# thodson-usgs/discontinuum

Measured on AMD Instinct MI355X. Metric: GP fits/sec (NLL+grad step) at n=8192 d=3, 1/2/4/8 MI355X, higher is better.
Workload: dtype f64

## Files before the change

### discontinuum_amd/_lib.py

```python
from __future__ import annotations

import ctypes as C
import os

_HERE = os.path.dirname(os.path.abspath(__file__))
LIB_PATH = os.path.join(_HERE, "libdgp_hip.so")

F64, F32 = 0, 1
MODEL_LOADEST, MODEL_RATING = 0, 1
OUT_NLL, OUT_QUAD, OUT_LOGDET, OUT_INFO, OUT_DTHETA, OUT_SUM_DR, OUT_DR_W0, OUT_SUM_DNOISE, OUT_LEN = 0, 1, 2, 3, 4, 28, 29, 31, 32
BUF_XT, BUF_A, BUF_T, BUF_S, BUF_Z, BUF_ALPHA = range(6)
BUF_INFO, BUF_SCAL = 6, 7
LCV_PLANE_NAMES = ("mu", "var", "lpd", "pit_lower", "pit_upper", "dlp", "tilt")
OPT_LAUUM64_MAX_TILES, OPT_SYRK_SLOTS, OPT_TRTRI_SMALL, OPT_REFINE, OPT_SYRK_ORDER, OPT_LAUUM_ORDER, OPT_CHAIN_YIELD, OPT_FUSED_GRAD, OPT_GROUP_GEMM = range(9)
OPT_POTRF_SCHEDULE, OPT_POTRF_SWEEP, OPT_POTRF_SOLVE, OPT_POTRF_OVERLAP, OPT_POTRF_SLOTS, OPT_POTRF_TAIL, OPT_POTRF_TAIL_SWEEP = range(9, 16)
TIME_GRAM, TIME_POTRF, TIME_SYRK_SUM, TIME_SYRK_N, TIME_TRTRI, TIME_LAUUM, TIME_SOLVE, TIME_GRAD, TIME_SYRK_FLOP, TIME_COUNT = range(10)


E_ARG, E_MODEL, E_WORKSPACE, E_STATE, E_FULL, E_NOCONV = -1, -2, -3, -4, -5, -6


class DGPLibraryError(RuntimeError):
    pass

# ... 89 lines not shown
    "dgp_predict_sensitivity_workspace_bytes": (_sz, [_vp, _i64, _i, _i]),
    "dgp_predict_sensitivity": (_i, [_vp, _dp, _vp, _i64, _vp, _i, _vp, _i, _vp, _sz, _vp, _vp, _vp]),
    "dgp_deletion_influence_workspace_bytes": (_sz, [_vp, _i64, _i, _i64, _i]),
    "dgp_deletion_influence": (_i, [_vp, _dp, _vp, _i64, _vp, _vp, _i, _i64, _i, _vp, _vp, _vp, _i, _vp, _vp, _sz, _vp, _vp, _vp, _vp, _vp]),
    "dgp_model_nterms": (_i, [_i, _i]),
    "dgp_predict_terms_workspace_bytes": (_sz, [_vp, _i64]),
    "dgp_predict_terms": (_i, [_vp, _dp, _vp, _i64, _vp, _sz, _vp, _vp, _vp]),
    "dgp_model_input_differentiable": (_i, [_i, _i, _i]),
    "dgp_predict_slopes_workspace_bytes": (_sz, [_vp, _i64, _i]),
    "dgp_predict_slopes": (_i, [_vp, _dp, _vp, _i64, C.POINTER(_i), _i, _vp, _sz, _vp, _vp, _vp]),
    "dgp_mean_vjp_workspace_bytes": (_sz, [_vp, _i64]),
    "dgp_predict_mean": (_i, [_vp, _dp, _vp, _i64, _vp, _sz, _vp, _vp]),
    "dgp_mean_vjp": (_i, [_vp, _dp, _vp, _i64, _vp, _vp, _sz, _vp, _vp, _vp, _vp]),
    "dgp_plan_set_timing": (_i, [_vp, _i]),
    "dgp_plan_get_timing": (_i, [_vp, _dp]),
    "dgp_stage_gram": (_i, [_vp, _dp, _vp, _vp]),
    "dgp_stage_potrf": (_i, [_vp, _vp]),
    "dgp_stage_trtri": (_i, [_vp, _vp]),
    "dgp_stage_lauum": (_i, [_vp, _vp]),
    "dgp_stage_solve": (_i, [_vp, _vp, _vp]),
    "dgp_stage_grad": (_i, [_vp, _dp, _vp, _vp]),
    "dgp_cross_gram": (_i, [_vp, _dp, _vp, _i64, _vp, _vp, _vp]),
    "dgp_debug_clock_probe": (_i, [_vp, _i, C.c_double, _vp]),
    "dgp_debug_tile_gemm": (_i, [_i, _i, _i, _i, _vp, _i64, _vp, _i64, _i64, _vp, _i64, _i, _i, _i, _i, _vp]),
}

_lib = None


def load():
    global _lib
    if _lib is not None:
        return _lib
    if not os.path.exists(LIB_PATH):
        raise DGPLibraryError(
            f"{LIB_PATH} not found: build it with `python -c 'import __graft_entry__ as g; g.build()'` "
            "or `make -C discontinuum_amd/csrc` (there is no CPU fallback)"
        )
    try:
        lib = C.CDLL(LIB_PATH)
    except OSError as e:
        raise DGPLibraryError(f"could not load {LIB_PATH}: {e}") from e
    for name, (res, args) in SIGNATURES.items():
        fn = getattr(lib, name)
        fn.restype = res
        fn.argtypes = args
# ... 10 lines not shown
```

### discontinuum_amd/csrc/dgp_chol.hip

```cpp
#include <stdlib.h>
#include <string.h>
#include <algorithm>
#include <mutex>
#include "dgp_diag.h"
#include "dgp_gemm.h"
#include "dgp_gemm_dma.h"
#include "dgp_internal.h"
#include "dgp_schedule.h"

namespace dgp {

static constexpr int NB = DGP_TILE;
static constexpr int SMID_TABLE = 4096;
template <typename T>
struct Prefetch {
  static constexpr bool F64 = sizeof(T) == 8;
  static constexpr int LAUUM = F64 ? 2 : 4, TRTRI = F64 ? 1 : 4, SYRK = F64 ? 1 : 2;
};

#define DGP_INFO_CHAIN_TIMEOUT (-7)
#define CHAIN_WAIT_TICKS 200000000LL
__device__ __forceinline__ bool chain_reached(const int* word, int value) {
  return __hip_atomic_load(word, __ATOMIC_RELAXED, __HIP_MEMORY_SCOPE_AGENT) >= value;
}
// ... 913 lines not shown
  G::foreach (acc, [&](int r, int c, T& v) { out[(long)r * ld + c] = v; });
}

template <typename T>
int lauum(const T* Tm, long N, T* S, hipStream_t s, Batch bt) {
  const int nbk = (int)(N / NB);
  const int tiles = nbk * (nbk + 1) / 2;
  if ((long)tiles * bt.B <= bt.tuning().lauum64_max_tiles) {
    const int nb64 = 2 * nbk;
    lauum64_kernel<T><<<dim3((unsigned)(nb64 * (nb64 + 1) / 2), 1, (unsigned)bt.B), 256, 0, s>>>(Tm, S, N, nb64, bt.ws);
  } else {
    const int sup = bt.tuning().lauum_super;
    unsigned grid = (unsigned)tiles;
    if (sup > 0) {
      const int nsr = (nbk + sup - 1) / sup, nst = nsr * (nsr + 1) / 2;
      grid = (unsigned)((nst + 7) / 8 * 8 * sup * sup);
    }
    lauum_kernel<T><<<dim3(grid, 1, (unsigned)bt.B), 256, 0, s>>>(Tm, S, N, nbk, bt.ws, sup);
  }
  return (int)hipGetLastError();
}

template <typename T>
__global__ __launch_bounds__(256) void trmv_n_kernel(const T* __restrict__ Tm, long ld, const T* __restrict__ r, int n,
                                                     T* __restrict__ z, long bs, const int* __restrict__ ns, long rs,
                                                     long zs = -1 ) {
  Tm = site(Tm, bs);
  z = site(z, zs >= 0 ? zs : bs);
  r = site(r, rs);
  n = site_n(ns, n);
  const int lane = threadIdx.x & 63;
  const long i = (long)blockIdx.x * 4 + (threadIdx.x >> 6);
  const long jend = (i / NB + 1) * NB;
  const T* row = Tm + i * ld;
  T acc = T(0);
  for (long j = lane; j < jend; j += 64) acc += row[j] * (j < n ? r[j] : T(0));
  acc = wave_sum(acc);
  if (lane == 0) z[i] = acc;
}

#define DGP_TRMV_CHUNK 512
static inline int trmv_chunk(long N) { return N < 2048 ? 128 : DGP_TRMV_CHUNK; }
template <typename T>
__global__ __launch_bounds__(256) void trmv_t_kernel(const T* __restrict__ Tm, long ld, const T* __restrict__ z,
                                                     T* __restrict__ partial, long bs, int chunk, long zs = -1) {
  Tm = site(Tm, bs);
  z = site(z, zs >= 0 ? zs : bs);
  partial = site(partial, zs >= 0 ? zs : bs);
  __shared__ T red[4][64];
  const int tx = threadIdx.x & 63, ty = threadIdx.x >> 6;
  const long j = (long)blockIdx.x * 64 + tx;
  const long r0 = (long)blockIdx.y * chunk, r1 = min(r0 + (long)chunk, ld);
  const long rstart = max(r0, ((long)blockIdx.x * 64 / NB) * NB);
  T acc = T(0);
  for (long i = rstart + ty; i < r1; i += 4) acc += Tm[i * ld + j] * z[i];
  red[ty][tx] = acc;
  __syncthreads();
  if (ty == 0) partial[(long)blockIdx.y * ld + j] = red[0][tx] + red[1][tx] + red[2][tx] + red[3][tx];
}

template <typename T>
__global__ __launch_bounds__(256) void trmv_t_reduce_kernel(const T* __restrict__ partial, long N, int nchunks,
                                                            T* __restrict__ alpha, long bs, int chunk,
                                                            const T* __restrict__ z, T* __restrict__ quad, long as = -1,
                                                            long zs = -1 ) {
  if (zs >= 0) bs = zs;
  if (blockIdx.x == gridDim.x - 1) {
    if (quad == nullptr) return;
    z = site(z, bs);
    quad = site(quad, bs);
    __shared__ double red[256];
    double acc = 0.0;
    for (long i = threadIdx.x; i < N; i += 256) acc += (double)z[i] * (double)z[i];
    red[threadIdx.x] = acc;
    __syncthreads();
    for (int s = 128; s > 0; s >>= 1) {
      if ((int)threadIdx.x < s) red[threadIdx.x] += red[threadIdx.x + s];
      __syncthreads();
    }
    if (threadIdx.x == 0) {
      quad[0] = (T)red[0];
      if (sizeof(T) == 4) *reinterpret_cast<double*>(quad + 3) = red[0];
    }
    return;
  }
  partial = site(partial, bs);
  alpha = site(alpha, as >= 0 ? as : bs);
  const long j = (long)blockIdx.x * 256 + threadIdx.x;
  if (j >= N) return;
  T acc = T(0);
  const int c0 = (int)((j / NB) * NB / chunk);
  for (int c = c0; c < nchunks; ++c) acc += partial[(long)c * N + j];
  alpha[j] = acc;
}

template <typename T>
__global__ __launch_bounds__(256) void symv_row_kernel(const T* __restrict__ S, long ld, const T* __restrict__ g,
                                                       T* __restrict__ out, long bs, long wbs) {
  S = site(S, bs);
  g = site(g, wbs);
  out = site(out, wbs);
  const int lane = threadIdx.x & 63;
  const long i = (long)blockIdx.x * 4 + (threadIdx.x >> 6);
  const T* row = S + i * ld;
  T acc = T(0);
  for (long j = lane; j <= i; j += 64) acc += row[j] * g[j];
  acc = wave_sum(acc);
  if (lane == 0) out[i] = acc;
}
template <typename T>
__global__ __launch_bounds__(256) void symv_col_kernel(const T* __restrict__ S, long ld, const T* __restrict__ g,
                                                       T* __restrict__ partial, long bs, long wbs) {
  S = site(S, bs);
  g = site(g, wbs);
  partial = site(partial, wbs);
  __shared__ T red[4][64];
  const int tx = threadIdx.x & 63, ty = threadIdx.x >> 6;
  const long j = (long)blockIdx.x * 64 + tx;
// ... 17 lines not shown
  n = site_n(ns, n);
  const long j = (long)blockIdx.x * 256 + threadIdx.x;
  if (j >= N) return;
  T acc = beta[j];
  for (int c = (int)(j / DGP_TRMV_CHUNK); c < nchunks; ++c) acc += partial[(long)c * N + j];
  acc = j < n ? acc : T(0);
  beta[j] = acc;
  if (j < nfull && dnoise) dnoise[j] = j < n ? -acc * alpha[j] : T(0);
}

template <typename T>
int symv_lower(const T* S, long N, const T* g, int n, const T* alpha, T* beta, T* partials, T* dnoise, hipStream_t s,
               Batch bt, long wbs) {
  const int nchunks = (int)((N + DGP_TRMV_CHUNK - 1) / DGP_TRMV_CHUNK);
  const unsigned Bz = (unsigned)bt.B;
  symv_row_kernel<T><<<dim3((unsigned)(N / 4), 1, Bz), 256, 0, s>>>(S, N, g, beta, bt.ws, wbs);
  dim3 grid((unsigned)(N / 64), (unsigned)nchunks, Bz);
  symv_col_kernel<T><<<grid, 256, 0, s>>>(S, N, g, partials, bt.ws, wbs);
  symv_finish_kernel<T><<<dim3((unsigned)((N + 255) / 256), 1, Bz), 256, 0, s>>>(partials, N, nchunks, alpha, n, beta, dnoise, bt.ws,
                                                                                wbs, bt.ns);
  return (int)hipGetLastError();
}

long solve_partials(long N) { return (N + trmv_chunk(N) - 1) / trmv_chunk(N) * N; }

template <typename T>
static void solve_pair(const T* Tm, long N, const T* r, long rs, int n, T* z, T* out, long os, T* partials, T* quad, hipStream_t s,
                       const Batch& bt) {
  const unsigned Bz = (unsigned)bt.B;
  trmv_n_kernel<T><<<dim3((unsigned)(N / 4), 1, Bz), 256, 0, s>>>(Tm, N, r, n, z, bt.ws, bt.ns, rs);
  const int chunk = trmv_chunk(N), nchunks = (int)((N + chunk - 1) / chunk);
  dim3 grid((unsigned)(N / 64), (unsigned)nchunks, Bz);
  trmv_t_kernel<T><<<grid, 256, 0, s>>>(Tm, N, z, partials, bt.ws, chunk);
  trmv_t_reduce_kernel<T><<<dim3((unsigned)((N + 255) / 256) + 1, 1, Bz), 256, 0, s>>>(partials, N, nchunks, out, bt.ws, chunk, z, quad, os);
}
template <typename T>
int solve(const T* Tm, long N, const T* r, int n, T* z, T* alpha, T* partials, T* quad, hipStream_t s, Batch bt) {
  solve_pair<T>(Tm, N, r, (long)n, n, z, alpha, -1, partials, quad, s, bt);
  return (int)hipGetLastError();
}
template <typename T>
int solve_work(const T* Tm, long N, const T* r, int n, T* z, T* out, T* partials, T* quad, long wss, hipStream_t s, Batch bt) {
  const unsigned Bz = (unsigned)bt.B;
  trmv_n_kernel<T><<<dim3((unsigned)(N / 4), 1, Bz), 256, 0, s>>>(Tm, N, r, n, z, bt.ws, bt.ns, wss, wss);
  const int chunk = trmv_chunk(N), nchunks = (int)((N + chunk - 1) / chunk);
  dim3 grid((unsigned)(N / 64), (unsigned)nchunks, Bz);
  trmv_t_kernel<T><<<grid, 256, 0, s>>>(Tm, N, z, partials, bt.ws, chunk, wss);
  trmv_t_reduce_kernel<T><<<dim3((unsigned)((N + 255) / 256) + 1, 1, Bz), 256, 0, s>>>(partials, N, nchunks, out, bt.ws, chunk, z, quad, wss,
                                                                                      wss);
  return (int)hipGetLastError();
}

template <typename T>
__global__ __launch_bounds__(256) void refine_finish_kernel(T* __restrict__ alpha, const T* __restrict__ delta,
                                                            const double* __restrict__ rho, const T* __restrict__ r, int n,
                                                            T* __restrict__ quad, long bs, long ps, long rs,
                                                            const int* __restrict__ ns) {
  alpha = site(alpha, bs);
  quad = site(quad, bs);
  delta = site(delta, rs);
  rho = site(rho, ps);
  r = site(r, (long)n);
  n = site_n(ns, n);
  __shared__ double red[256];
  double acc = 0.0;
  for (long i = threadIdx.x; i < n; i += 256) {
    const double a0 = (double)alpha[i], a1 = a0 + (double)delta[i];
    acc += (double)r[i] * a0 + rho[i] * a1;
    alpha[i] = (T)a1;
  }
  red[threadIdx.x] = acc;
  __syncthreads();
  for (int s = 128; s > 0; s >>= 1) {
    if ((int)threadIdx.x < s) red[threadIdx.x] += red[threadIdx.x + s];
    __syncthreads();
  }
  if (threadIdx.x == 0) {
    quad[0] = (T)red[0];
    if (sizeof(T) == 4) *reinterpret_cast<double*>(quad + 3) = red[0];
  }
}

template <typename T>
int refine_solve(const T* Tm, long N, const T* r, int n, const double* rho64, const T* rho32, T* z, T* delta, T* alpha,
                 T* partials, T* quad, hipStream_t s, Batch bt, long ps, long rs) {
  solve_pair<T>(Tm, N, rho32, rs, n, z, delta, rs, partials, nullptr, s, bt);
  refine_finish_kernel<T><<<dim3(1, 1, (unsigned)bt.B), 256, 0, s>>>(alpha, delta, rho64, r, n, quad, bt.ws, ps, rs, bt.ns);
  return (int)hipGetLastError();
}

template <typename T>
__global__ __launch_bounds__(256, (TileCore<T, true, false>::OCC)) void predict_v_kernel(const T* __restrict__ Tm, long N, const T* __restrict__ Ks,
                                                        long M, T* __restrict__ V, long bs, long wbs) {
  Tm = site(Tm, bs);
  Ks = site(Ks, wbs);
  V = site(V, wbs);
  using K = TileCore<T, true, false>;
  using G = typename K::G;
  __shared__ T smem[K::SMEM_ELEMS];
  const int bi = gridDim.y - 1 - blockIdx.y, bj = blockIdx.x;
  typename G::acc_t acc[G::MI][G::NI];
  G::zero(acc);
  K::run(Tm + (long)bi * NB * N, N, Ks + (long)bj * NB, M, (bi + 1) * (NB / 16), smem, acc);
  T* out = V + (long)bi * NB * M + (long)bj * NB;
  G::foreach (acc, [&](int r, int c, T& v) { out[(long)r * M + c] = v; });
}

template <typename T>
__global__ __launch_bounds__(256) void predict_partial_kernel(const T* __restrict__ V, const T* __restrict__ Ks, long N,
// ... 104 lines not shown
    const long q = (long)bq * NB + r, j = (long)bj * NB + c;
    if (q < ndraw && j < m) out[q * m + j] = v + (mean ? mean[j] : T(0));
  });
}

template <typename T>
int sample_draws(const T* L, long M, const T* Z, long Q, const T* mean, int m, int ndraw, T* out, hipStream_t s) {
  sample_draws_kernel<T><<<dim3((unsigned)(Q / NB), (unsigned)(M / NB)), 256, 0, s>>>(L, M, Z, Q, mean, m, ndraw, out);
  return (int)hipGetLastError();
}

#define DGP_INST(T)                                                                                              \
  template int posterior_cov<T>(const T*, long, long, T*, hipStream_t, int, long);                                          \
  template int posterior_cov_panel<T>(const T*, long, long, T*, long, long, long, hipStream_t, int, long);                                          \
  template int sample_draws<T>(const T*, long, const T*, long, const T*, int, int, T*, hipStream_t);             \
  template int symv_lower<T>(const T*, long, const T*, int, const T*, T*, T*, T*, hipStream_t, Batch, long);     \
  template int potrf<T>(T*, long, T*, T*, int*, int, hipStream_t, hipStream_t, hipEvent_t*, PotrfObservers*, Batch, int);               \
  template int potrf_split<T>(T*, long, T*, T*, int*, T*, hipStream_t, hipStream_t, hipStream_t, hipEvent_t*, PotrfObservers*, int, int,  \
                              const Tuning*);                                                                                             \
  template int potrf_group<T>(T*, long, int, T*, T*, int*, int, int, hipStream_t);                                \
  template int trtri_advance<T>(const T*, long, T*, T*, int, TrtriProgress*, hipStream_t, int, int*, int, int, Batch, long);                   \
  template int trtri<T>(const T*, const T*, long, T*, T*, hipStream_t, Batch, long);                                        \
  template int lauum<T>(const T*, long, T*, hipStream_t, Batch);                                                      \
  template int solve<T>(const T*, long, const T*, int, T*, T*, T*, T*, hipStream_t, Batch);                           \
  template int solve_work<T>(const T*, long, const T*, int, T*, T*, T*, T*, long, hipStream_t, Batch);                \
  template int refine_solve<T>(const T*, long, const T*, int, const double*, const T*, T*, T*, T*, T*, T*, hipStream_t, Batch, long, long); \
  template int predict_v<T>(const T*, long, const T*, long, T*, hipStream_t, Batch, long);                                  \
  template int predict_var<T>(const T*, long, const T*, long, T*, const T*, const T*, T*, T*, T*, hipStream_t, Batch, long);
DGP_INST(double)
DGP_INST(float)

}

#ifdef DGP_DIAG_LOG
extern "C" int dgp_debug_diag_log(unsigned long long* out_host) {
  return (int)hipMemcpyFromSymbol(out_host, HIP_SYMBOL(dgp::dgp_diag_log), sizeof(unsigned long long) * 4 * 1024);
}
#endif
```

### discontinuum_amd/csrc/dgp_gram.hip

```cpp
#include <mutex>
#include <string.h>
#include "dgp_internal.h"
#include "dgp_models.h"
#include "dgp_gram_shared.h"

namespace dgp {

size_t pre_scratch_bytes(int B) { return B > DGP_MAX_BATCH ? (size_t)B * DGP_PRE_SLOT_BYTES : 0; }

#define DGP_C_MAXMODELS 64
static CompositeDesc g_comp[DGP_C_MAXMODELS];
static int g_ncomp = 0;
static std::mutex g_comp_mtx;
static thread_local const CompositeDesc* g_comp_cur = nullptr;
const CompositeDesc* composite_current() { return g_comp_cur; }
static const CompositeDesc* composite_get(int model) {
  const int slot = model - DGP_MODEL_COMPOSITE_BASE;
  return (slot >= 0 && slot < g_ncomp) ? &g_comp[slot] : nullptr;
}
bool composite_select(int model, int d) {
  g_comp_cur = composite_get(model);
  return g_comp_cur && g_comp_cur->d == d;
}

// ... 168 lines not shown
    }
    store4<T>(Ks + gi * Mp + (long)bj * 64 + tx * 4, out);
  }
}

template <typename T, typename M>
__global__ __launch_bounds__(256) void gram_diag_kernel(const T* __restrict__ Xst, long Mp, int m, const PreBatch<M> pb,
                                                        T* __restrict__ kss, long wbs) {
  const typename M::Pre& pre = pb.get();
  Xst = site(Xst, wbs);
  kss = site(kss, wbs);
  exp_table_init<T>();
  __syncthreads();
  const long j = (long)blockIdx.x * 256 + threadIdx.x;
  if (j >= Mp) return;
  T x[M::NX], f[M::NF], dummy[M::NTHETA];
#pragma unroll
  for (int c = 0; c < M::NX; ++c) x[c] = Xst[(long)c * Mp + j];
  M::features(x, pre, f);
  T v = M::template pair<false>(f, f, pre, T(0), dummy);
  kss[j] = j < m ? v : T(0);
}

template <typename T, typename M, int MODE>
__global__ __launch_bounds__(256) void gram_grad_kernel(const T* __restrict__ Xt, long N, int n, const PreBatch<M> pb,
                                                        const T* __restrict__ S, const T* __restrict__ alpha,
                                                        const T* __restrict__ beta, T* __restrict__ partials, long bs,
                                                        const int* __restrict__ ns, long wbs ) {
  n = site_n(ns, n);
  const typename M::Pre& pre = pb.get();
  Xt = site(Xt, bs);
  if (MODE == 0) S = site(S, bs);
  alpha = site(alpha, bs);
  partials = site(partials, MODE == 0 ? bs : wbs);
  if (MODE == 1) beta = site(beta, wbs);
  __shared__ T sfi[M::NF][64], sfj[M::NF][64], sai[64], saj[64], sbi[64], sbj[64];
  __shared__ T red[4][M::NTHETA];
  int bi, bj;
  tri_decode(blockIdx.x, bi, bj);
  const int t = threadIdx.x;
  exp_table_init<T>();
  if (t < 64) {
    stage_strip<T, M>(Xt, N, (long)bi * 64, pre, sfi, t);
    sai[t] = alpha[(long)bi * 64 + t];
    sbi[t] = MODE == 1 ? beta[(long)bi * 64 + t] : T(0);
  } else if (t < 128) {
    stage_strip<T, M>(Xt, N, (long)bj * 64, pre, sfj, t - 64);
    saj[t - 64] = alpha[(long)bj * 64 + t - 64];
    sbj[t - 64] = MODE == 1 ? beta[(long)bj * 64 + t - 64] : T(0);
  }
  __syncthreads();
  const int ty = t >> 4, tx = t & 15;
  T acc[M::NTHETA];
#pragma unroll
  for (int p = 0; p < M::NTHETA; ++p) acc[p] = T(0);
#pragma unroll 1
  for (int a = 0; a < 4; ++a) {
    const long gi = (long)bi * 64 + ty * 4 + a;
    T fi[M::NF];
#pragma unroll
    for (int c = 0; c < M::NF; ++c) fi[c] = sfi[c][ty * 4 + a];
    const T ai = sai[ty * 4 + a], bi_ = sbi[ty * 4 + a];
    T sv[4] = {T(0), T(0), T(0), T(0)};
    if (MODE == 0) load4<T>(S + gi * N + (long)bj * 64 + tx * 4, sv);
#pragma unroll 1
    for (int b = 0; b < 4; ++b) {
      const int cj = tx * 4 + b;
      const long gj = (long)bj * 64 + cj;
      T fj[M::NF];
#pragma unroll
      for (int c = 0; c < M::NF; ++c) fj[c] = sfj[c][cj];
      const T aj = saj[cj];
      const T svb = b == 0 ? sv[0] : (b == 1 ? sv[1] : (b == 2 ? sv[2] : sv[3]));
      T w = MODE == 0 ? svb - ai * aj : -(bi_ * aj + sbj[cj] * ai);
      w = (gj > gi || gi >= n) ? T(0) : (gj == gi ? T(0.5) * w : w);
      (void)M::template pair<true>(fi, fj, pre, w, acc);
    }
  }
  M::finalize(acc, pre);
  const int lane = t & 63, wv = t >> 6;
#pragma unroll
  for (int p = 0; p < M::NTHETA; ++p) {
    T v = wave_sum(acc[p]);
    if (lane == 0) red[wv][p] = v;
  }
  __syncthreads();
  if (t < M::NTHETA) partials[(long)blockIdx.x * DGP_MAX_THETA + t] = red[0][t] + red[1][t] + red[2][t] + red[3][t];
}

template <typename T, typename M>
__global__ __launch_bounds__(256) void gram_cross_grad_kernel(const T* __restrict__ Xt, long N, int n,
                                                              const T* __restrict__ Xst, long Mp, int m,
                                                              const PreBatch<M> pb, const T* __restrict__ alpha,
                                                              const T* __restrict__ wts, T* __restrict__ partials, long bs,
                                                              long wbs, const int* __restrict__ ns) {
  const typename M::Pre& pre = pb.get();
  Xt = site(Xt, bs);
  alpha = site(alpha, bs);
  Xst = site(Xst, wbs);
  partials = site(partials, wbs);
// ... 316 lines not shown

template <typename T>
int gram_diag(int model, int d, const T* Xst, long Mp, int m, const double* theta, T* kss, hipStream_t s, Batch bt, long wbs,
              void* pre_scratch) {
  const int nt = model_ntheta(model, d);
  if (nt < 0) return -2;
  dim3 grid((unsigned)((Mp + 255) / 256), 1, (unsigned)bt.B);
  DGP_DISPATCH_MODEL(model, d, (gram_diag_kernel<T, M><<<grid, dim3(256), 0, s>>>(
                                   Xst, Mp, m, prepare_batch<M>(theta, nt, bt.B, pre_scratch, false, s), kss, wbs)));
  return (int)hipGetLastError();
}

long gram_grad_partials(long N) {
  const long nb = N / 64;
  return nb * (nb + 1) / 2 * DGP_MAX_THETA;
}

template <typename T>
int gram_grad(int model, int d, const T* Xt, long N, int n, const double* theta, const T* S, const T* alpha,
              T* partials, T* dtheta, hipStream_t s, Batch bt, long dtheta_stride, void* pre_scratch, bool pre_ready,
              void* pre_staging) {
  const int nt = model_ntheta(model, d);
  if (nt < 0) return -2;
  const long nb = N / 64;
  const long nblk = nb * (nb + 1) / 2;
  DGP_DISPATCH_MODEL(model, d,
                     (gram_grad_kernel<T, M, 0><<<dim3((unsigned)nblk, 1, (unsigned)bt.B), dim3(256), 0, s>>>(
                         Xt, N, n, prepare_batch<M>(theta, nt, bt.B, pre_scratch, !pre_ready, s, pre_staging), S, alpha, nullptr,
                         partials, bt.ws, bt.ns, 0)));
  grad_reduce_kernel<T><<<dim3((unsigned)nt, 1, (unsigned)bt.B), dim3(256), 0, s>>>(partials, nblk, nt, dtheta, 0, bt.ws,
                                                                                 dtheta_stride);
  return (int)hipGetLastError();
}

template <typename T>
int mean_vjp_grad(int model, int d, const T* Xt, long N, int n, const T* Xst, long Mp, int m, const double* theta,
                  const T* alpha, const T* beta, const T* wts, T* partials, T* dtheta, hipStream_t s, Batch bt, long wbs,
                  long dstride, void* pre_scratch, void* pre_staging) {
  const int nt = model_ntheta(model, d);
  if (nt < 0) return -2;
  const long nb = N / 64;
  const long nblk = nb * (nb + 1) / 2;
  const unsigned Bz = (unsigned)bt.B;
  DGP_DISPATCH_MODEL(model, d,
                     (gram_grad_kernel<T, M, 1><<<dim3((unsigned)nblk, 1, Bz), dim3(256), 0, s>>>(
                         Xt, N, n, prepare_batch<M>(theta, nt, bt.B, pre_scratch, true, s, pre_staging), nullptr, alpha, beta, partials,
                         bt.ws, bt.ns, wbs)));
  grad_reduce_kernel<T><<<dim3((unsigned)nt, 1, Bz), dim3(256), 0, s>>>(partials, nblk, nt, dtheta, 0, wbs, dstride);
  dim3 grid((unsigned)(Mp / 64), (unsigned)(N / 64), Bz);
  DGP_DISPATCH_MODEL(model, d,
                     (gram_cross_grad_kernel<T, M><<<grid, dim3(256), 0, s>>>(
                         Xt, N, n, Xst, Mp, m, prepare_batch<M>(theta, nt, bt.B, pre_scratch, false, s), alpha, wts, partials, bt.ws, wbs,
                         bt.ns)));
  grad_reduce_kernel<T><<<dim3((unsigned)nt, 1, Bz), dim3(256), 0, s>>>(partials, (long)grid.x * grid.y, nt, dtheta, 1, wbs, dstride);
  return (int)hipGetLastError();
}

template <typename T>
int gram_slab(int model, int d, const T* Xt, long N, int n, const double* theta, const T* noise, T* Aslab, long Cl,
              SlabMap sm, hipStream_t s) {
  if (model_ntheta(model, d) < 0) return -2;
  dim3 grid((unsigned)(N / 64), (unsigned)(Cl / 64));
  DGP_DISPATCH_MODEL(model, d, (gram_slab_kernel<T, M><<<grid, dim3(256), 0, s>>>(Xt, N, n, M::prepare(theta), noise, Aslab, Cl, sm)));
  return (int)hipGetLastError();
}
// ... 64 lines not shown
```

### discontinuum_amd/csrc/dgp_internal.h

```cpp
#pragma once
#include <hip/hip_runtime.h>
#include <stdint.h>

#define DGP_TILE_HOST 128

namespace dgp {

inline long round_up(long n, long q) { return (n + q - 1) / q * q; }

#define DGP_MAX_BATCH_HOST 8
#define DGP_MAX_BATCH_SITES 1024
struct Tuning {
  int lauum64_max_tiles;
  int syrk_slots;
  long trtri_small;
  int syrk_super;
  int lauum_super;
  int chain_yield;
  int fused_grad;
  int group_gemm;
  int potrf_schedule;
  int potrf_sweep;
  int potrf_tail;
  int potrf_tail_sweep;
// ... 97 lines not shown
  static constexpr int MAXLVL = 16;
  int wdone[MAXLVL] = {0}, gdone[MAXLVL] = {0};
  int pairs_used = 0;
};
template <typename T>
int trtri_advance(const T* L, long N, T* Tm, T* W, int ready_blocks, TrtriProgress* st, hipStream_t s, int wg_cap,
                  int* ctr , int nctr_pairs, int reserve_cus, Batch bt = Batch(),
                  long ld = 0 );
#define CHAIN_FLAG0 2
#define EARLY_CTR0 4
#define EARLY_CTR_PAIRS 125
#define POTRF_INFO_INTS (EARLY_CTR0 + 2 * EARLY_CTR_PAIRS + 4)
#define CHAIN_ABORT (POTRF_INFO_INTS - 4)
#define CHAIN_YIELD (POTRF_INFO_INTS - 3)
#define CHAIN_DIAG_DONE (POTRF_INFO_INTS - 2)
#define CHAIN_TICKET (POTRF_INFO_INTS - 1)
const unsigned char* reserved_cu_table(int nreserve, int* n_cu);
template <typename T>
int trtri(const T* L, const T* Dinv, long N, T* Tm, T* W, hipStream_t s, Batch bt = Batch(), long ld = 0);
template <typename T>
int lauum(const T* Tm, long N, T* S, hipStream_t s, Batch bt = Batch());
template <typename T>
int solve(const T* Tm, long N, const T* r, int n, T* z, T* alpha, T* partials, T* quad, hipStream_t s,
          Batch bt = Batch());
template <typename T>
int refine_solve(const T* Tm, long N, const T* r, int n, const double* rho64, const T* rho32, T* z, T* delta, T* alpha,
                 T* partials, T* quad, hipStream_t s, Batch bt, long scratch_stride ,
                 long rho32_stride );
#define PREDICT_SPLIT 32
template <typename T>
int predict_var(const T* Tm, long N, const T* Ks, long M, T* V, const T* alpha, const T* kss, T* part, T* mean, T* var,
                hipStream_t s, Batch bt = Batch(), long wbs = 0);
template <typename T>
int predict_v(const T* Tm, long N, const T* Ks, long M, T* V, hipStream_t s, Batch bt = Batch(), long wbs = 0);
template <typename T>
int solve_work(const T* Tm, long N, const T* r, int n, T* z, T* out, T* partials, T* quad, long wss, hipStream_t s, Batch bt = Batch());
long solve_partials(long N);
template <typename T>
int potrf_group(T* A, long ld, int nbk, T* Tinv, T* logdet, int* info, int k0, int W, hipStream_t s);
struct SlabMap {
  int W, world, rank;
  __host__ __device__ int gblock(int lb) const { return ((lb / W) * world + rank) * W + lb % W; }
};
template <typename T>
int gram_slab(int model, int d, const T* Xt, long N, int n, const double* theta, const T* noise, T* Aslab, long Cl,
              SlabMap sm, hipStream_t s);
template <typename T>
// ... 207 lines not shown
```

### discontinuum_amd/csrc/dgp_selftest.hip

```cpp
#include "../../include/dgp_hip.h"
#include "dgp_gemm.h"
#include "dgp_gemm_dma.h"

namespace dgp {

template <typename T, bool AKC, bool BKC, bool DMA, int VARIANT>
__global__ __launch_bounds__(256, (TileCore<T, AKC, BKC, 128, 128, 1, DMA>::OCC)) void tile_gemm_kernel(
    const T* __restrict__ A, long lda, const T* __restrict__ B, long ldb, int ktiles, T* __restrict__ C, long ldc, int reverse) {
  using K = TileCore<T, AKC, BKC, 128, 128, 1, DMA, (VARIANT > 0)>;
  using G = typename K::G;
  __shared__ T smem[K::SMEM_ELEMS];
  const int bm = blockIdx.y, bn = blockIdx.x;
  typename G::acc_t acc[G::MI][G::NI];
  G::zero(acc);
  const T* a = AKC ? A + (long)bm * 128 * lda : A + (long)bm * 128;
  const T* b = BKC ? B + (long)bn * 128 * ldb : B + (long)bn * 128;
  constexpr int TRI = VARIANT >= 2 ? VARIANT - 1 : 0;
  T* out = C + (long)bm * 128 * ldc + (long)bn * 128;
  auto store = [&]() { K::foreach (acc, [&](int r, int c, T& v) { out[(long)r * ldc + c] = v; }); };
  if (reverse) K::template run_tri<true, TRI>(a, lda, b, ldb, ktiles, smem, acc, store);
  else K::template run_tri<false, TRI>(a, lda, b, ldb, ktiles, smem, acc, store);
}

template <typename T, bool DMA, int VARIANT>
static int launch(int a_kc, int b_kc, const T* A, long lda, const T* B, long ldb, int ktiles, T* C, long ldc, dim3 grid,
// ... 17 lines not shown
    default: return launch<T, true, 5>(a_kc, b_kc, A, lda, B, ldb, ktiles, C, ldc, grid, s, rev);
  }
}

}

extern "C" int dgp_debug_tile_gemm(int dtype, int core, int a_kc, int b_kc, const void* A, int64_t lda, const void* B,
                                   int64_t ldb, int64_t k, void* C, int64_t ldc, int tiles_m, int tiles_n, int reverse,
                                   int variant, void* stream) {
  using namespace dgp;
  if (variant < 0 || variant > 5 || (variant > 0 && core != 1) || (variant >= 2 && k % 128 != 0)) return DGP_E_ARG;
  if ((dtype != DGP_F64 && dtype != DGP_F32) || (core != 0 && core != 1) || !A || !B || !C || k < 16 || k % 16 != 0 ||
      k > (1 << 24) || tiles_m < 1 || tiles_n < 1 || tiles_m > 4096 || tiles_n > 4096 || lda < 1 || ldb < 1 || ldc < 128L * tiles_n)
    return DGP_E_ARG;
  const int64_t epu = dtype == DGP_F64 ? 2 : 4;
  if (lda % epu || ldb % epu || ((uintptr_t)A & 15) || ((uintptr_t)B & 15)) return DGP_E_ARG;
  const dim3 grid((unsigned)tiles_n, (unsigned)tiles_m);
  hipStream_t s = (hipStream_t)stream;
  const int kt = (int)(k / 16);
  if (dtype == DGP_F64)
    return launch_variant<double>(core, variant, a_kc, b_kc, (const double*)A, lda, (const double*)B, ldb, kt, (double*)C, ldc, grid, s, reverse);
  return launch_variant<float>(core, variant, a_kc, b_kc, (const float*)A, lda, (const float*)B, ldb, kt, (float*)C, ldc, grid, s, reverse);
}
```

### include/dgp_hip.h

```cpp
#ifndef DGP_HIP_H
#define DGP_HIP_H
#include <stddef.h>
#include <stdint.h>

#ifdef __cplusplus
extern "C" {
#endif

#define DGP_F64 0
#define DGP_F32 1
#define DGP_MODEL_LOADEST 0
#define DGP_MODEL_RATING 1

#define DGP_E_ARG (-1)
#define DGP_E_MODEL (-2)
#define DGP_E_WORKSPACE (-3)
#define DGP_E_STATE (-4)
#define DGP_E_FULL (-5)
#define DGP_E_NOCONV (-6)

#define DGP_OUT_NLL 0
#define DGP_OUT_QUAD 1
#define DGP_OUT_LOGDET 2
#define DGP_OUT_INFO 3
// ... 220 lines not shown
int dgp_dist_residual(dgp_dist* h, const double* theta_host, const void* noise_dev, const void* r_dev, const void* alpha_dev,
                      double* rho64_dev, void* rho32_dev, void* stream);
int dgp_dist_pack_inverse(dgp_dist* h, int group, void* panel_dev, void* stream);
int dgp_dist_product(dgp_dist* h, int group, const void* panel_dev, void* stream);
int dgp_dist_grad_partial(dgp_dist* h, const double* theta_host, const void* alpha_dev, void* dtheta_part_dev,
                          void* dnoise_part_dev, void* stream);
int dgp_dist_slab(const dgp_dist* h, int which, void** dev_ptr);

int dgp_stage_gram(dgp_plan* plan, const double* theta_host, const void* noise_dev, void* stream);
int dgp_stage_potrf(dgp_plan* plan, void* stream);
int dgp_stage_trtri(dgp_plan* plan, void* stream);
int dgp_stage_lauum(dgp_plan* plan, void* stream);
int dgp_stage_solve(dgp_plan* plan, const void* r_dev, void* stream);
int dgp_stage_grad(dgp_plan* plan, const double* theta_host, void* dtheta_dev, void* stream);
int dgp_cross_gram(dgp_plan* plan, const double* theta_host, const void* Xs_dev, int64_t m, void* work_dev,
                   void* Ks_dev, void* stream);

int dgp_debug_tile_gemm(int dtype, int core, int a_kc, int b_kc, const void* A_dev, int64_t lda, const void* B_dev,
                        int64_t ldb, int64_t k, void* C_dev, int64_t ldc, int tiles_m, int tiles_n, int reverse, int variant,
                        void* stream);

int dgp_debug_clock_probe(void* out_dev, int nwg, double seconds, void* stream);

#ifdef __cplusplus
}
#endif
#endif
```

Measured before the change: 114.8.

## Fuse two-pass triangular solve into a single row kernel; batch grad tiles

The old solve used three kernels: a row-wise trmv, a chunked transposed trmv and a reduce. These are replaced by one kernel that reads each row of the inverse factor once, using buffer loads and double-buffered row pairs. It computes z_i and accumulates the transposed product into per-group partials, and a lighter kernel then reduces the partials. Separately, the gradient Gram kernel now gives each block a run of up to eight column tiles sharing one row strip, with a branch-free interior path. This cuts staging work and launch block count. The trade-off is more shared memory, a fixed group count that limits parallelism, and an f64 path that rejects large N needing the tail.

```diff
diff --git a/discontinuum_amd/_lib.py b/discontinuum_amd/_lib.py
--- a/discontinuum_amd/_lib.py
+++ b/discontinuum_amd/_lib.py
@@ -135,6 +135,8 @@
     "dgp_stage_grad": (_i, [_vp, _dp, _vp, _vp]),
     "dgp_cross_gram": (_i, [_vp, _dp, _vp, _i64, _vp, _vp, _vp]),
     "dgp_debug_clock_probe": (_i, [_vp, _i, C.c_double, _vp]),
+    "dgp_debug_solve": (_i, [_i, _i, _vp, _i64, _vp, _i64, _vp, _vp, _vp, _vp, _vp]),
+    "dgp_debug_solve_partials": (_i64, [_i64]),
     "dgp_debug_tile_gemm": (_i, [_i, _i, _i, _i, _vp, _i64, _vp, _i64, _i64, _vp, _i64, _i, _i, _i, _i, _vp]),
 }
 
diff --git a/discontinuum_amd/csrc/dgp_chol.hip b/discontinuum_amd/csrc/dgp_chol.hip
--- a/discontinuum_amd/csrc/dgp_chol.hip
+++ b/discontinuum_amd/csrc/dgp_chol.hip
@@ -959,48 +959,148 @@
 }
 
 template <typename T>
-__global__ __launch_bounds__(256) void trmv_n_kernel(const T* __restrict__ Tm, long ld, const T* __restrict__ r, int n,
-                                                     T* __restrict__ z, long bs, const int* __restrict__ ns, long rs,
-                                                     long zs = -1 ) {
+__device__ __forceinline__ T wave_sum_all(T v) {
+  constexpr int NWORD = sizeof(T) / 4;
+  union U {
+    T t;
+    int w[NWORD];
+  };
+#define DGP_SWZ_STEP(XOR)                                                                         \
+  {                                                                                               \
+    U a, b;                                                                                       \
+    a.t = v;                                                                                      \
+    _Pragma("unroll") for (int q = 0; q < NWORD; ++q) b.w[q] = __builtin_amdgcn_ds_swizzle(a.w[q], ((XOR) << 10) | 0x1f); \
+    v += b.t;                                                                                     \
+  }
+  DGP_SWZ_STEP(16) DGP_SWZ_STEP(8) DGP_SWZ_STEP(4) DGP_SWZ_STEP(2) DGP_SWZ_STEP(1)
+#undef DGP_SWZ_STEP
+  U a, lo, hi;
+  a.t = v;
+#pragma unroll
+  for (int q = 0; q < NWORD; ++q) {
+    lo.w[q] = __builtin_amdgcn_readlane(a.w[q], 0);
+    hi.w[q] = __builtin_amdgcn_readlane(a.w[q], 32);
+  }
+  return lo.t + hi.t;
+}
+#define DGP_SOLVE_KT(T) (int)(sizeof(T) == 8 ? 8 : 4)
+#define DGP_SOLVE_NT 512
+template <typename T>
+struct alignas(16) SolvePack {
+  T e[16 / sizeof(T)];
+};
+template <typename T, int KT, bool RL, bool TAIL>
+__global__ __launch_bounds__(DGP_SOLVE_NT, RL ? 4 : 2) void trsv_rows_kernel(const T* __restrict__ Tm, long ld, const T* __restrict__ r, int n,
+                                                           T* __restrict__ z, T* __restrict__ partial, long bs,
+                                                           const int* __restrict__ ns, long rs, long zs, int G) {
+  using P = SolvePack<T>;
+  constexpr int W = 16 / sizeof(T), NT = DGP_SOLVE_NT, NW = NT / 64, SEG = NT * W;
+  constexpr long CAP = (long)KT * SEG;
+  extern __shared__ __attribute__((aligned(16))) unsigned char trsv_smem[];
+  T* red = reinterpret_cast<T*>(trsv_smem);
+  T* rl = reinterpret_cast<T*>(trsv_smem + 128);
   Tm = site(Tm, bs);
   z = site(z, zs >= 0 ? zs : bs);
+  partial = site(partial, zs >= 0 ? zs : bs) + (long)blockIdx.x * ld;
   r = site(r, rs);
   n = site_n(ns, n);
-  const int lane = threadIdx.x & 63;
-  const long i = (long)blockIdx.x * 4 + (threadIdx.x >> 6);
-  const long jend = (i / NB + 1) * NB;
-  const T* row = Tm + i * ld;
-  T acc = T(0);
-  for (long j = lane; j < jend; j += 64) acc += row[j] * (j < n ? r[j] : T(0));
-  acc = wave_sum(acc);
-  if (lane == 0) z[i] = acc;
-}
-
-#define DGP_TRMV_CHUNK 512
-static inline int trmv_chunk(long N) { return N < 2048 ? 128 : DGP_TRMV_CHUNK; }
-template <typename T>
-__global__ __launch_bounds__(256) void trmv_t_kernel(const T* __restrict__ Tm, long ld, const T* __restrict__ z,
-                                                     T* __restrict__ partial, long bs, int chunk, long zs = -1) {
-  Tm = site(Tm, bs);
-  z = site(z, zs >= 0 ? zs : bs);
-  partial = site(partial, zs >= 0 ? zs : bs);
-  __shared__ T red[4][64];
-  const int tx = threadIdx.x & 63, ty = threadIdx.x >> 6;
-  const long j = (long)blockIdx.x * 64 + tx;
-  const long r0 = (long)blockIdx.y * chunk, r1 = min(r0 + (long)chunk, ld);
-  const long rstart = max(r0, ((long)blockIdx.x * 64 / NB) * NB);
-  T acc = T(0);
-  for (long i = rstart + ty; i < r1; i += 4) acc += Tm[i * ld + j] * z[i];
-  red[ty][tx] = acc;
-  __syncthreads();
-  if (ty == 0) partial[(long)blockIdx.y * ld + j] = red[0][tx] + red[1][tx] + red[2][tx] + red[3][tx];
-}
-
-template <typename T>
-__global__ __launch_bounds__(256) void trmv_t_reduce_kernel(const T* __restrict__ partial, long N, int nchunks,
-                                                            T* __restrict__ alpha, long bs, int chunk,
-                                                            const T* __restrict__ z, T* __restrict__ quad, long as = -1,
-                                                            long zs = -1 ) {
+  const int tid = threadIdx.x, lane = tid & 63, wv = tid >> 6;
+  const long j0 = (long)tid * W;
+  const long rlen = ld > CAP ? (ld + SEG - 1) / SEG * SEG : CAP;
+  if (RL) {
+    for (long j = tid; j < rlen; j += NT) rl[j] = j < n ? r[j] : T(0);
+    __syncthreads();
+  }
+  auto rvec = [&](long j) {
+    P v;
+    if (RL) {
+      v = *reinterpret_cast<const P*>(rl + j);
+    } else {
+#pragma unroll
+      for (int e = 0; e < W; ++e) v.e[e] = j + e < n ? r[j + e] : T(0);
+    }
+    return v;
+  };
+  P acc[KT];
+#pragma unroll
+  for (int k = 0; k < KT; ++k)
+#pragma unroll
+    for (int e = 0; e < W; ++e) acc[k].e[e] = T(0);
+  for (long j = CAP + j0; TAIL && j < ld; j += SEG) *reinterpret_cast<P*>(partial + j) = acc[0];
+
+  const int voff = (int)(j0 * (long)sizeof(T));
+  auto load = [&](P(&v)[KT], long i) {
+    const long jend = (i / NB + 1) * NB;
+    const long jreg = jend < CAP ? jend : CAP;
+    const auto rsrc = __builtin_amdgcn_make_buffer_rsrc(const_cast<T*>(Tm + i * ld), 0, (int)(jreg * (long)sizeof(T)), 0x00020000);
+#pragma unroll
+    for (int k = 0; k < KT; ++k)
+      v[k] = __builtin_bit_cast(P, __builtin_amdgcn_raw_buffer_load_b128(rsrc, voff + k * SEG * (int)sizeof(T), 0, 0));
+  };
+  auto consume = [&](const P(&v)[KT], long i, int par) {
+    const long jend = (i / NB + 1) * NB;
+    const T* row = Tm + i * ld;
+    T d = T(0);
+#pragma unroll
+    for (int k = 0; k < KT; ++k) {
+      const P rr = rvec(j0 + (long)k * SEG);
+#pragma unroll
+      for (int e = 0; e < W; ++e) d += v[k].e[e] * rr.e[e];
+      __builtin_amdgcn_sched_barrier(0);
+    }
+    for (long j = CAP + j0; TAIL && j < jend; j += SEG) {
+      const P t = *reinterpret_cast<const P*>(row + j), rr = rvec(j);
+#pragma unroll
+      for (int e = 0; e < W; ++e) d += t.e[e] * rr.e[e];
+    }
+    d = wave_sum_all(d);
+    if (lane == 0) red[par * NW + wv] = d;
+    __syncthreads();
+    T zi = T(0);
+#pragma unroll
+    for (int w = 0; w < NW; ++w) zi += red[par * NW + w];
+    if (tid == 0) z[i] = zi;
+#pragma unroll
+    for (int k = 0; k < KT; ++k)
+#pragma unroll
+      for (int e = 0; e < W; ++e) acc[k].e[e] += zi * v[k].e[e];
+    for (long j = CAP + j0; TAIL && j < jend; j += SEG) {
+      const P t = *reinterpret_cast<const P*>(row + j);
+      P a = *reinterpret_cast<P*>(partial + j);
+#pragma unroll
+      for (int e = 0; e < W; ++e) a.e[e] += zi * t.e[e];
+      *reinterpret_cast<P*>(partial + j) = a;
+    }
+  };
+
+  const long half = ld / 2;
+  auto rowat = [&](long m) {
+    const long p = (long)blockIdx.x + (m >> 1) * G;
+    return p < half ? ((m & 1) ? ld - 1 - p : p) : -1L;
+  };
+  P va[KT], vb[KT];
+  long m = 0, i = rowat(0), inext;
+  if (i >= 0) load(va, i);
+  while (i >= 0) {
+    if ((inext = rowat(m + 1)) >= 0) load(vb, inext);
+    consume(va, i, 0);
+    if ((i = inext) < 0) break;
+    if ((inext = rowat(m + 2)) >= 0) load(va, inext);
+    consume(vb, i, 1);
+    i = inext;
+    m += 2;
+  }
+#pragma unroll
+  for (int k = 0; k < KT; ++k)
+    if (j0 + (long)k * SEG < ld) *reinterpret_cast<P*>(partial + j0 + (long)k * SEG) = acc[k];
+}
+
+static inline int solve_groups(long N) { return (int)(N / 4 < 128 ? N / 4 : 128); }
+
+template <typename T>
+__global__ __launch_bounds__(256) void trsv_reduce_kernel(const T* __restrict__ partial, long N, int G, T* __restrict__ alpha,
+                                                          long bs, const T* __restrict__ z, T* __restrict__ quad, long as = -1,
+                                                          long zs = -1 ) {
   if (zs >= 0) bs = zs;
   if (blockIdx.x == gridDim.x - 1) {
     if (quad == nullptr) return;
@@ -1023,14 +1123,17 @@
   }
   partial = site(partial, bs);
   alpha = site(alpha, as >= 0 ? as : bs);
-  const long j = (long)blockIdx.x * 256 + threadIdx.x;
-  if (j >= N) return;
+  __shared__ T part[4][64];
+  const int tx = threadIdx.x & 63, ty = threadIdx.x >> 6;
+  const long j = (long)blockIdx.x * 64 + tx;
   T acc = T(0);
-  const int c0 = (int)((j / NB) * NB / chunk);
-  for (int c = c0; c < nchunks; ++c) acc += partial[(long)c * N + j];
-  alpha[j] = acc;
-}
-
+  for (int g = ty; g < G; g += 4) acc += partial[(long)g * N + j];
+  part[ty][tx] = acc;
+  __syncthreads();
+  if (ty == 0) alpha[j] = (part[0][tx] + part[1][tx]) + (part[2][tx] + part[3][tx]);
+}
+
+#define DGP_TRMV_CHUNK 512
 template <typename T>
 __global__ __launch_bounds__(256) void symv_row_kernel(const T* __restrict__ S, long ld, const T* __restrict__ g,
                                                        T* __restrict__ out, long bs, long wbs) {
@@ -1094,33 +1197,49 @@
   return (int)hipGetLastError();
 }
 
-long solve_partials(long N) { return (N + trmv_chunk(N) - 1) / trmv_chunk(N) * N; }
-
-template <typename T>
-static void solve_pair(const T* Tm, long N, const T* r, long rs, int n, T* z, T* out, long os, T* partials, T* quad, hipStream_t s,
-                       const Batch& bt) {
-  const unsigned Bz = (unsigned)bt.B;
-  trmv_n_kernel<T><<<dim3((unsigned)(N / 4), 1, Bz), 256, 0, s>>>(Tm, N, r, n, z, bt.ws, bt.ns, rs);
-  const int chunk = trmv_chunk(N), nchunks = (int)((N + chunk - 1) / chunk);
-  dim3 grid((unsigned)(N / 64), (unsigned)nchunks, Bz);
-  trmv_t_kernel<T><<<grid, 256, 0, s>>>(Tm, N, z, partials, bt.ws, chunk);
-  trmv_t_reduce_kernel<T><<<dim3((unsigned)((N + 255) / 256) + 1, 1, Bz), 256, 0, s>>>(partials, N, nchunks, out, bt.ws, chunk, z, quad, os);
-}
-template <typename T>
-int solve(const T* Tm, long N, const T* r, int n, T* z, T* alpha, T* partials, T* quad, hipStream_t s, Batch bt) {
-  solve_pair<T>(Tm, N, r, (long)n, n, z, alpha, -1, partials, quad, s, bt);
+static inline long symv_chunks(long N) { return (N + DGP_TRMV_CHUNK - 1) / DGP_TRMV_CHUNK; }
+long solve_partials(long N) { return (solve_groups(N) > symv_chunks(N) ? solve_groups(N) : symv_chunks(N)) * N; }
+
+template <typename T, int KT, bool RL, bool TAIL>
+static int launch_trsv_rows(const T* Tm, long N, const T* r, int n, T* z, T* partials, long rs, long zs, int G, hipStream_t s,
+                            const Batch& bt) {
+  constexpr long SEG = DGP_SOLVE_NT * 16 / (long)sizeof(T), CAP = KT * SEG;
+  const size_t bytes = 128 + (RL ? (size_t)(N > CAP ? (N + SEG - 1) / SEG * SEG : CAP) * sizeof(T) : 0);
+  if (bytes > 64 * 1024) {
+    static DeviceOnce configured;
+    (void)configured.run([&] {
+      return hipFuncSetAttribute(reinterpret_cast<const void*>(&trsv_rows_kernel<T, KT, RL, TAIL>),
+                                 hipFuncAttributeMaxDynamicSharedMemorySize, 128 + 64 * 1024);
+    });
+  }
+  trsv_rows_kernel<T, KT, RL, TAIL><<<dim3((unsigned)G, 1, (unsigned)bt.B), DGP_SOLVE_NT, bytes, s>>>(Tm, N, r, n, z, partials, bt.ws, bt.ns, rs, zs, G);
   return (int)hipGetLastError();
 }
 template <typename T>
+static int solve_pair(const T* Tm, long N, const T* r, long rs, int n, T* z, T* out, long os, T* partials, T* quad, long zs,
+                      hipStream_t s, const Batch& bt, int kt = 0) {
+  const int G = solve_groups(N);
+  const bool rl = (size_t)N * sizeof(T) <= 64 * 1024;
+  constexpr int KT = DGP_SOLVE_KT(T);
+  const bool tail = N > (long)KT * DGP_SOLVE_NT * 16 / (long)sizeof(T);
+  int rc;
+  if (kt == 1) rc = rl ? launch_trsv_rows<T, 1, true, true>(Tm, N, r, n, z, partials, rs, zs, G, s, bt)
+                       : launch_trsv_rows<T, 1, false, true>(Tm, N, r, n, z, partials, rs, zs, G, s, bt);
+  else if (!rl) rc = launch_trsv_rows<T, KT, false, true>(Tm, N, r, n, z, partials, rs, zs, G, s, bt);
+  else if (!tail) rc = launch_trsv_rows<T, KT, true, false>(Tm, N, r, n, z, partials, rs, zs, G, s, bt);
+  else if constexpr (sizeof(T) == 4) rc = launch_trsv_rows<T, KT, true, true>(Tm, N, r, n, z, partials, rs, zs, G, s, bt);
+  else return (int)hipErrorInvalidValue;
+  if (rc) return rc;
+  trsv_reduce_kernel<T><<<dim3((unsigned)(N / 64) + 1, 1, (unsigned)bt.B), 256, 0, s>>>(partials, N, G, out, bt.ws, z, quad, os, zs);
+  return (int)hipGetLastError();
+}
+template <typename T>
+int solve(const T* Tm, long N, const T* r, int n, T* z, T* alpha, T* partials, T* quad, hipStream_t s, Batch bt, int kt) {
+  return solve_pair<T>(Tm, N, r, (long)n, n, z, alpha, -1, partials, quad, -1, s, bt, kt);
+}
+template <typename T>
 int solve_work(const T* Tm, long N, const T* r, int n, T* z, T* out, T* partials, T* quad, long wss, hipStream_t s, Batch bt) {
-  const unsigned Bz = (unsigned)bt.B;
-  trmv_n_kernel<T><<<dim3((unsigned)(N / 4), 1, Bz), 256, 0, s>>>(Tm, N, r, n, z, bt.ws, bt.ns, wss, wss);
-  const int chunk = trmv_chunk(N), nchunks = (int)((N + chunk - 1) / chunk);
-  dim3 grid((unsigned)(N / 64), (unsigned)nchunks, Bz);
-  trmv_t_kernel<T><<<grid, 256, 0, s>>>(Tm, N, z, partials, bt.ws, chunk, wss);
-  trmv_t_reduce_kernel<T><<<dim3((unsigned)((N + 255) / 256) + 1, 1, Bz), 256, 0, s>>>(partials, N, nchunks, out, bt.ws, chunk, z, quad, wss,
-                                                                                      wss);
-  return (int)hipGetLastError();
+  return solve_pair<T>(Tm, N, r, wss, n, z, out, wss, partials, quad, wss, s, bt);
 }
 
 template <typename T>
@@ -1156,7 +1275,7 @@
 template <typename T>
 int refine_solve(const T* Tm, long N, const T* r, int n, const double* rho64, const T* rho32, T* z, T* delta, T* alpha,
                  T* partials, T* quad, hipStream_t s, Batch bt, long ps, long rs) {
-  solve_pair<T>(Tm, N, rho32, rs, n, z, delta, rs, partials, nullptr, s, bt);
+  if (int rc = solve_pair<T>(Tm, N, rho32, rs, n, z, delta, rs, partials, nullptr, -1, s, bt)) return rc;
   refine_finish_kernel<T><<<dim3(1, 1, (unsigned)bt.B), 256, 0, s>>>(alpha, delta, rho64, r, n, quad, bt.ws, ps, rs, bt.ns);
   return (int)hipGetLastError();
 }
@@ -1307,7 +1426,7 @@
   template int trtri_advance<T>(const T*, long, T*, T*, int, TrtriProgress*, hipStream_t, int, int*, int, int, Batch, long);                   \
   template int trtri<T>(const T*, const T*, long, T*, T*, hipStream_t, Batch, long);                                        \
   template int lauum<T>(const T*, long, T*, hipStream_t, Batch);                                                      \
-  template int solve<T>(const T*, long, const T*, int, T*, T*, T*, T*, hipStream_t, Batch);                           \
+  template int solve<T>(const T*, long, const T*, int, T*, T*, T*, T*, hipStream_t, Batch, int);                           \
   template int solve_work<T>(const T*, long, const T*, int, T*, T*, T*, T*, long, hipStream_t, Batch);                \
   template int refine_solve<T>(const T*, long, const T*, int, const double*, const T*, T*, T*, T*, T*, T*, hipStream_t, Batch, long, long); \
   template int predict_v<T>(const T*, long, const T*, long, T*, hipStream_t, Batch, long);                                  \
diff --git a/discontinuum_amd/csrc/dgp_gram.hip b/discontinuum_amd/csrc/dgp_gram.hip
--- a/discontinuum_amd/csrc/dgp_gram.hip
+++ b/discontinuum_amd/csrc/dgp_gram.hip
@@ -214,6 +214,20 @@
   kss[j] = j < m ? v : T(0);
 }
 
+#define DGP_GRAD_RUN 8
+__device__ __forceinline__ void grad_run_decode(int idx, int& bi, int& run) {
+  int q = (int)((sqrtf((float)idx + 1.0f) - 1.0f) * 0.5f);
+  while ((DGP_GRAD_RUN / 2) * (q + 1) * (q + 2) <= idx) ++q;
+  while ((DGP_GRAD_RUN / 2) * q * (q + 1) > idx) --q;
+  const int rem = idx - (DGP_GRAD_RUN / 2) * q * (q + 1);
+  bi = DGP_GRAD_RUN * q + rem / (q + 1);
+  run = rem % (q + 1);
+}
+static long grad_runs(long nb) {
+  long total = 0;
+  for (long bi = 0; bi < nb; ++bi) total += bi / DGP_GRAD_RUN + 1;
+  return total;
+}
 template <typename T, typename M, int MODE>
 __global__ __launch_bounds__(256) void gram_grad_kernel(const T* __restrict__ Xt, long N, int n, const PreBatch<M> pb,
                                                         const T* __restrict__ S, const T* __restrict__ alpha,
@@ -226,48 +240,61 @@
   alpha = site(alpha, bs);
   partials = site(partials, MODE == 0 ? bs : wbs);
   if (MODE == 1) beta = site(beta, wbs);
-  __shared__ T sfi[M::NF][64], sfj[M::NF][64], sai[64], saj[64], sbi[64], sbj[64];
+  __shared__ T sfi[M::NF][64], sfj[DGP_GRAD_RUN][M::NF][64], sai[64], saj[DGP_GRAD_RUN][64], sbi[64], sbj[DGP_GRAD_RUN][64];
   __shared__ T red[4][M::NTHETA];
-  int bi, bj;
-  tri_decode(blockIdx.x, bi, bj);
+  int bi, run;
+  grad_run_decode(blockIdx.x, bi, run);
+  const int bj0 = run * DGP_GRAD_RUN, bj1 = min(bj0 + DGP_GRAD_RUN, bi + 1);
   const int t = threadIdx.x;
   exp_table_init<T>();
-  if (t < 64) {
-    stage_strip<T, M>(Xt, N, (long)bi * 64, pre, sfi, t);
-    sai[t] = alpha[(long)bi * 64 + t];
-    sbi[t] = MODE == 1 ? beta[(long)bi * 64 + t] : T(0);
-  } else if (t < 128) {
-    stage_strip<T, M>(Xt, N, (long)bj * 64, pre, sfj, t - 64);
-    saj[t - 64] = alpha[(long)bj * 64 + t - 64];
-    sbj[t - 64] = MODE == 1 ? beta[(long)bj * 64 + t - 64] : T(0);
+  for (int strip = t >> 6; strip <= bj1 - bj0; strip += 4) {
+    const int l = t & 63;
+    if (strip == 0) {
+      stage_strip<T, M>(Xt, N, (long)bi * 64, pre, sfi, l);
+      sai[l] = alpha[(long)bi * 64 + l];
+      sbi[l] = MODE == 1 ? beta[(long)bi * 64 + l] : T(0);
+    } else {
+      const long base = (long)(bj0 + strip - 1) * 64;
+      stage_strip<T, M>(Xt, N, base, pre, sfj[strip - 1], l);
+      saj[strip - 1][l] = alpha[base + l];
+      sbj[strip - 1][l] = MODE == 1 ? beta[base + l] : T(0);
+    }
   }
   __syncthreads();
   const int ty = t >> 4, tx = t & 15;
   T acc[M::NTHETA];
 #pragma unroll
   for (int p = 0; p < M::NTHETA; ++p) acc[p] = T(0);
+  auto tile = [&](auto interior, int bj, int buf) {
+    constexpr bool INTERIOR = decltype(interior)::value;
 #pragma unroll 1
-  for (int a = 0; a < 4; ++a) {
-    const long gi = (long)bi * 64 + ty * 4 + a;
-    T fi[M::NF];
-#pragma unroll
-    for (int c = 0; c < M::NF; ++c) fi[c] = sfi[c][ty * 4 + a];
-    const T ai = sai[ty * 4 + a], bi_ = sbi[ty * 4 + a];
-    T sv[4] = {T(0), T(0), T(0), T(0)};
-    if (MODE == 0) load4<T>(S + gi * N + (long)bj * 64 + tx * 4, sv);
+    for (int a = 0; a < 4; ++a) {
+      const long gi = (long)bi * 64 + ty * 4 + a;
+      T fi[M::NF];
+#pragma unroll
+      for (int c = 0; c < M::NF; ++c) fi[c] = sfi[c][ty * 4 + a];
+      const T ai = sai[ty * 4 + a], bi_ = sbi[ty * 4 + a];
+      T sv[4] = {T(0), T(0), T(0), T(0)};
+      if (MODE == 0) load4<T>(S + gi * N + (long)bj * 64 + tx * 4, sv);
 #pragma unroll 1
-    for (int b = 0; b < 4; ++b) {
-      const int cj = tx * 4 + b;
-      const long gj = (long)bj * 64 + cj;
-      T fj[M::NF];
-#pragma unroll
-      for (int c = 0; c < M::NF; ++c) fj[c] = sfj[c][cj];
-      const T aj = saj[cj];
-      const T svb = b == 0 ? sv[0] : (b == 1 ? sv[1] : (b == 2 ? sv[2] : sv[3]));
-      T w = MODE == 0 ? svb - ai * aj : -(bi_ * aj + sbj[cj] * ai);
-      w = (gj > gi || gi >= n) ? T(0) : (gj == gi ? T(0.5) * w : w);
-      (void)M::template pair<true>(fi, fj, pre, w, acc);
-    }
+      for (int b = 0; b < 4; ++b) {
+        const int cj = tx * 4 + b;
+        const long gj = (long)bj * 64 + cj;
+        T fj[M::NF];
+#pragma unroll
+        for (int c = 0; c < M::NF; ++c) fj[c] = sfj[buf][c][cj];
+        const T aj = saj[buf][cj];
+        const T svb = b == 0 ? sv[0] : (b == 1 ? sv[1] : (b == 2 ? sv[2] : sv[3]));
+        T w = MODE == 0 ? svb - ai * aj : -(bi_ * aj + sbj[buf][cj] * ai);
+        if (!INTERIOR) w = (gj > gi || gi >= n) ? T(0) : (gj == gi ? T(0.5) * w : w);
+        (void)M::template pair<true>(fi, fj, pre, w, acc);
+      }
+    }
+  };
+  const bool rows_real = ((long)bi + 1) * 64 <= n;
+  for (int bj = bj0; bj < bj1; ++bj) {
+    if (rows_real && bj < bi) tile(std::true_type{}, bj, bj - bj0);
+    else tile(std::false_type{}, bj, bj - bj0);
   }
   M::finalize(acc, pre);
   const int lane = t & 63, wv = t >> 6;
@@ -630,8 +657,7 @@
               void* pre_staging) {
   const int nt = model_ntheta(model, d);
   if (nt < 0) return -2;
-  const long nb = N / 64;
-  const long nblk = nb * (nb + 1) / 2;
+  const long nblk = grad_runs(N / 64);
   DGP_DISPATCH_MODEL(model, d,
                      (gram_grad_kernel<T, M, 0><<<dim3((unsigned)nblk, 1, (unsigned)bt.B), dim3(256), 0, s>>>(
                          Xt, N, n, prepare_batch<M>(theta, nt, bt.B, pre_scratch, !pre_ready, s, pre_staging), S, alpha, nullptr,
@@ -647,8 +673,7 @@
                   long dstride, void* pre_scratch, void* pre_staging) {
   const int nt = model_ntheta(model, d);
   if (nt < 0) return -2;
-  const long nb = N / 64;
-  const long nblk = nb * (nb + 1) / 2;
+  const long nblk = grad_runs(N / 64);
   const unsigned Bz = (unsigned)bt.B;
   DGP_DISPATCH_MODEL(model, d,
                      (gram_grad_kernel<T, M, 1><<<dim3((unsigned)nblk, 1, Bz), dim3(256), 0, s>>>(
diff --git a/discontinuum_amd/csrc/dgp_internal.h b/discontinuum_amd/csrc/dgp_internal.h
--- a/discontinuum_amd/csrc/dgp_internal.h
+++ b/discontinuum_amd/csrc/dgp_internal.h
@@ -143,7 +143,7 @@
 int lauum(const T* Tm, long N, T* S, hipStream_t s, Batch bt = Batch());
 template <typename T>
 int solve(const T* Tm, long N, const T* r, int n, T* z, T* alpha, T* partials, T* quad, hipStream_t s,
-          Batch bt = Batch());
+          Batch bt = Batch(), int kt = 0 );
 template <typename T>
 int refine_solve(const T* Tm, long N, const T* r, int n, const double* rho64, const T* rho32, T* z, T* delta, T* alpha,
                  T* partials, T* quad, hipStream_t s, Batch bt, long scratch_stride ,
diff --git a/discontinuum_amd/csrc/dgp_selftest.hip b/discontinuum_amd/csrc/dgp_selftest.hip
--- a/discontinuum_amd/csrc/dgp_selftest.hip
+++ b/discontinuum_amd/csrc/dgp_selftest.hip
@@ -1,6 +1,7 @@
 #include "../../include/dgp_hip.h"
 #include "dgp_gemm.h"
 #include "dgp_gemm_dma.h"
+#include "dgp_internal.h"
 
 namespace dgp {
 
@@ -64,3 +65,20 @@
     return launch_variant<double>(core, variant, a_kc, b_kc, (const double*)A, lda, (const double*)B, ldb, kt, (double*)C, ldc, grid, s, reverse);
   return launch_variant<float>(core, variant, a_kc, b_kc, (const float*)A, lda, (const float*)B, ldb, kt, (float*)C, ldc, grid, s, reverse);
 }
+
+extern "C" int64_t dgp_debug_solve_partials(int64_t N) {
+  return (N < 128 || N % 128 != 0 || N > 65536) ? (int64_t)DGP_E_ARG : (int64_t)dgp::solve_partials((long)N);
+}
+extern "C" int dgp_debug_solve(int dtype, int capacity, const void* Tm, int64_t N, const void* r, int64_t n, void* z, void* alpha,
+                               void* partials, void* quad, void* stream) {
+  using namespace dgp;
+  if ((dtype != DGP_F64 && dtype != DGP_F32) || (capacity != 0 && capacity != 1) || !Tm || !r || !z || !alpha || !partials || !quad ||
+      N < 128 || N % 128 != 0 || N > 65536 || n < 1 || n > N || ((uintptr_t)Tm & 15) || ((uintptr_t)partials & 15) || ((uintptr_t)quad & 7))
+    return DGP_E_ARG;
+  hipStream_t s = (hipStream_t)stream;
+  if (dtype == DGP_F64)
+    return solve<double>((const double*)Tm, (long)N, (const double*)r, (int)n, (double*)z, (double*)alpha, (double*)partials, (double*)quad, s,
+                         Batch(), capacity);
+  return solve<float>((const float*)Tm, (long)N, (const float*)r, (int)n, (float*)z, (float*)alpha, (float*)partials, (float*)quad + 1, s,
+                      Batch(), capacity);
+}
diff --git a/include/dgp_hip.h b/include/dgp_hip.h
--- a/include/dgp_hip.h
+++ b/include/dgp_hip.h
@@ -266,6 +266,10 @@
 
 int dgp_debug_clock_probe(void* out_dev, int nwg, double seconds, void* stream);
 
+int dgp_debug_solve(int dtype, int capacity, const void* Tm_dev, int64_t N, const void* r_dev, int64_t n, void* z_dev,
+                    void* alpha_dev, void* partials_dev, void* quad_dev, void* stream);
+int64_t dgp_debug_solve_partials(int64_t N);
+
 #ifdef __cplusplus
 }
 #endif
```

Result: faster. 116.7 (median of 6 runs) (+1.7%).
